# jonassibbesen/rpvg

Hardware: AMD Instinct MI355X
Metric: read-pairs quantified/sec (higher is better)
Workload: dtype f64

## Files before the change

rpvg_amd/csrc/bounded_search.hip:

```cpp

#include "common.hpp"
#include "search_plan.hpp"

#include <algorithm>
#include <cstdlib>
#include <map>
#include <memory>
#include <mutex>
#include <numeric>

using namespace rpvg_hip_detail;
using namespace rpvg_search;

namespace {
std::mutex g_search_gate_mutex;
const rpvg_hip_ctx * g_search_gate_owner = nullptr;
}

static bool searchLaunchesEarly() {
    static const bool early = RPVG_EXPERIMENT_ENV("RPVG_HIP_SEARCH_LAUNCH_EARLY") != nullptr;
    return early;
}

constexpr uint64_t kSearchGateRows = 1ull << 17;

static void searchGateEnter(rpvg_hip_ctx * ctx, hipStream_t stream, const uint64_t matrix_rows) {
    static const bool open_gate = RPVG_EXPERIMENT_ENV("RPVG_HIP_NO_SEARCH_GATE") != nullptr;
    ctx->search_gate_held = !open_gate && matrix_rows >= kSearchGateRows;
    if (!ctx->search_gate_held) return;
    hipEvent_t previous = nullptr;
    {
        std::lock_guard<std::mutex> lock(g_search_gate_mutex);
        if (g_search_gate_owner && g_search_gate_owner != ctx && g_search_gate_owner->device == ctx->device) {
            previous = g_search_gate_owner->search_done;
            (void) hipStreamWaitEvent(stream, previous, 0);
        }
    }
    if (previous && !searchLaunchesEarly()) (void) waitEvent(previous);
}

static void searchGateLeave(rpvg_hip_ctx * ctx, hipStream_t stream) {
    if (!ctx->search_gate_held) return;
    ctx->search_gate_held = false;
    std::lock_guard<std::mutex> lock(g_search_gate_mutex);
    (void) hipEventRecord(ctx->search_done, stream);
    g_search_gate_owner = ctx;
}

void searchGateForget(const rpvg_hip_ctx * ctx) {
    std::lock_guard<std::mutex> lock(g_search_gate_mutex);
    if (g_search_gate_owner == ctx) g_search_gate_owner = nullptr;
}

struct rpvg_hip_pair_posteriors {
    std::vector<uint64_t> pair_off;
    void * block = nullptr;
    bool block_pinned = false;
    const uint32_t * first = nullptr, * second = nullptr;
    const double * posterior = nullptr;
    ~rpvg_hip_pair_posteriors() {
        if (block && block_pinned) pinnedFree(block);
        else std::free(block);
    }
};

namespace {

constexpr uint32_t kLdsRows = 2048;
constexpr uint32_t kSmallRowLdsCols = 128;
constexpr uint32_t kRowLdsCols = 512;

// ... 1276 lines not shown
```

rpvg_amd/csrc/subset_em.hip:

```cpp

#include "common.hpp"
#include "subset_pack.hpp"

#include <cmath>
#include <memory>

using namespace rpvg_hip_detail;

namespace {

constexpr uint32_t kMaxSelected = 1024;

struct MergedList {
    const uint32_t * a;
    const uint32_t * b;
    uint32_t na, nb, i, j;
    __device__ __forceinline__ MergedList(const uint32_t * a_in, uint32_t na_in, const uint32_t * b_in, uint32_t nb_in)
        : a(a_in), b(b_in), na(na_in), nb(nb_in), i(0), j(0) {}
    __device__ __forceinline__ bool done() const { return i >= na && j >= nb; }
    __device__ __forceinline__ uint32_t next() {
        if (j >= nb || (i < na && a[i] <= b[j])) return a[i++];
        return b[j++];
    }
};

struct Columns {
    const uint64_t * group_path_off;
    const uint32_t * group_path;
    uint64_t first_column;
    __device__ __forceinline__ MergedList list(const uint32_t first, const uint32_t second) const {
        const uint64_t a0 = group_path_off[first_column + first], a1 = group_path_off[first_column + first + 1];
        const uint64_t b0 = group_path_off[first_column + second], b1 = group_path_off[first_column + second + 1];
        return MergedList(group_path + a0, static_cast<uint32_t>(a1 - a0), group_path + b0, static_cast<uint32_t>(b1 - b0));
    }
};
// ... 2 lines not shown
    while (!x.done() && !y.done()) {
        const uint32_t px = x.next(), py = y.next();
        if (px != py) return px < py ? -1 : 1;
    }
    if (x.done() && y.done()) return 0;
    return x.done() ? -1 : 1;
}

struct SelectArgs {
    uint32_t num_matrices;
    const uint32_t * pair_count;
    const uint64_t * pair_cap_off;
    const uint32_t * pair_first;
    const uint32_t * pair_second;
    const double * pair_value;
    const uint64_t * group_off;
    const uint64_t * group_path_off;
    const uint32_t * group_path;
    const uint32_t * cluster;
    const uint64_t * mat_rows;
    const uint64_t * cluster_row_off;
    const uint64_t * row_ent_off;
    const uint64_t * slot_off;
    double min_hap_prob;
    uint32_t segment_rows;
    uint32_t * slot_first;
    uint32_t * slot_second;
    double * slot_weight;
    uint32_t * slot_length;
    uint32_t * slot_columns;
    MatrixTotals * totals;
    SubsetHeader * header;
    uint32_t * big_matrices;
};

constexpr uint32_t kSmallSelected = 64;
constexpr uint32_t kSmallCachedPaths = 1024, kWideCachedPaths = 6144;

struct CachedColumns {
    const uint64_t * group_path_off;
    const uint32_t * paths;
    uint64_t first_column, base;
    __device__ __forceinline__ MergedList list(const uint32_t first, const uint32_t second) const {
        const uint64_t a0 = group_path_off[first_column + first], a1 = group_path_off[first_column + first + 1];
        const uint64_t b0 = group_path_off[first_column + second], b1 = group_path_off[first_column + second + 1];
        return MergedList(paths + (a0 - base), static_cast<uint32_t>(a1 - a0), paths + (b0 - base), static_cast<uint32_t>(b1 - b0));
    }
};

template <uint32_t CAP, uint32_t CACHE, int BLOCK>
__device__ __forceinline__ void selectSubsetsOfMatrix(const SelectArgs & args, const uint32_t m) {
    __shared__ uint32_t sel[CAP];
    __shared__ unsigned long long hash[CAP];
    __shared__ uint32_t length[CAP];
    __shared__ uint32_t leader[CAP];
    __shared__ double weight[CAP];
    __shared__ uint32_t order[CAP];
    __shared__ uint32_t cached_paths[CACHE];
    __shared__ uint32_t scratch[BLOCK / 64];
    __shared__ double sum_posterior;
    __shared__ unsigned long long red[3];
    __shared__ uint32_t n_retained;
    const uint32_t n_pairs = args.pair_count[m];
    const uint64_t base = args.pair_cap_off[m];
    const uint32_t * first = args.pair_first + base;
    const uint32_t * second = args.pair_second + base;
    const double * value = args.pair_value + base;
    const uint32_t k = args.cluster[m];
    MatrixTotals * out_totals = args.totals + m;
    const uint64_t col0 = args.group_off[m], col1 = args.group_off[m + 1];
    const uint64_t path0 = args.group_path_off[col0], path1 = args.group_path_off[col1];
    const bool cached = path1 - path0 <= CACHE;
    if (cached) {
        for (uint32_t i = threadIdx.x; i < path1 - path0; i += BLOCK) cached_paths[i] = args.group_path[path0 + i];
    }
    const CachedColumns columns{args.group_path_off, cached ? cached_paths : args.group_path, col0, cached ? path0 : 0};

    uint32_t n_sel = 0;
    for (uint32_t c = 0; c < n_pairs; c += BLOCK) {
        const uint32_t i = c + threadIdx.x;
        const uint32_t take = (i < n_pairs && value[i] >= args.min_hap_prob) ? 1u : 0u;
        uint32_t total;
        const uint32_t at = n_sel + blockExclusiveScan<BLOCK>(take, total, scratch);
        if (take && at < CAP) sel[at] = i;
        n_sel += total;
    }
    if (n_sel > CAP) {
        if (threadIdx.x == 0) {
            atomicAdd(&args.header->select_overflow, 1ull);
            *out_totals = MatrixTotals{0, 0, 0, 0, 0, 0};
        }
        return;
    }
    __syncthreads();
    if (threadIdx.x == 0) {
        double sum = 0;
        for (uint32_t s = 0; s < n_sel; ++s) sum += value[sel[s]];
        sum_posterior = sum;
        red[0] = red[1] = red[2] = 0;
        n_retained = 0;
    }
    for (uint32_t s = threadIdx.x; s < n_sel; s += BLOCK) {
        MergedList list = columns.list(first[sel[s]], second[sel[s]]);
        unsigned long long h = 1469598103934665603ull;
        uint32_t n = 0;
        while (!list.done()) {
            h = (h ^ list.next()) * 1099511628211ull;
            ++n;
        }
        hash[s] = h;
        length[s] = n;
    }
    __syncthreads();
    for (uint32_t s = threadIdx.x; s < n_sel; s += BLOCK) {
        uint32_t lead = s;
        for (uint32_t t = 0; t < s; ++t) {
            if (hash[t] == hash[s] && length[t] == length[s] &&
                compareLists(columns.list(first[sel[t]], second[sel[t]]), columns.list(first[sel[s]], second[sel[s]])) == 0) {
                lead = t;
                break;
            }
        }
        leader[s] = lead;
    }
    __syncthreads();
    for (uint32_t s = threadIdx.x; s < n_sel; s += BLOCK) {
        double w = 0;
        if (leader[s] == s) {
            for (uint32_t t = s; t < n_sel; ++t) {
                if (leader[t] == s) w += value[sel[t]];
            }
            w /= sum_posterior;
            if (w >= args.min_hap_prob) order[atomicAdd(&n_retained, 1u)] = s;
        }
        weight[s] = w;
    }
    __syncthreads();
    const uint32_t n_ret = n_retained;
    uint32_t padded = 1;
    while (padded < n_ret) padded <<= 1;
    for (uint32_t i = n_ret + threadIdx.x; i < padded; i += BLOCK) order[i] = 0xffffffffu;
    __syncthreads();
    auto before = [&](const uint32_t x, const uint32_t y) {
        if (x == 0xffffffffu) return false;
        if (y == 0xffffffffu) return true;
        return compareLists(columns.list(first[sel[x]], second[sel[x]]), columns.list(first[sel[y]], second[sel[y]])) < 0;
    };
    for (uint32_t size = 2; size <= padded; size <<= 1) {
        for (uint32_t stride = size >> 1; stride > 0; stride >>= 1) {
            for (uint32_t i = threadIdx.x; i < padded; i += BLOCK) {
                const uint32_t partner = i ^ stride;
                if (partner > i) {
                    const bool ascending = (i & size) == 0;
                    const uint32_t x = order[i], y = order[partner];
                    if (before(y, x) == ascending) {
                        order[i] = y;
                        order[partner] = x;
                    }
                }
            }
            __syncthreads();
        }
    }
    const uint64_t slot0 = args.slot_off[m];
    unsigned long long my_subsets = 0, my_length = 0, my_columns = 0;
    for (uint32_t rank = threadIdx.x; rank < n_ret; rank += BLOCK) {
        const uint32_t s = order[rank];
        uint32_t distinct = 0, previous = 0xffffffffu;
        MergedList walk = columns.list(first[sel[s]], second[sel[s]]);
        while (!walk.done()) {
            const uint32_t path = walk.next();
            distinct += (path != previous) ? 1u : 0u;
            previous = path;
        }
        args.slot_first[slot0 + rank] = first[sel[s]];
        args.slot_second[slot0 + rank] = second[sel[s]];
        args.slot_weight[slot0 + rank] = weight[s];
        args.slot_length[slot0 + rank] = length[s];
        args.slot_columns[slot0 + rank] = distinct;
        my_subsets += 1;
        my_length += length[s];
        my_columns += distinct;
    }
    if (my_subsets) {
        atomicAdd(&red[0], my_subsets);
        atomicAdd(&red[1], my_length);
        atomicAdd(&red[2], my_columns);
    }
    __syncthreads();
    if (threadIdx.x == 0) {
        const uint64_t r0 = args.cluster_row_off[k], r1 = args.cluster_row_off[k + 1];
        const unsigned long long rows = r1 - r0, entries = args.row_ent_off[r1] - args.row_ent_off[r0];
        *out_totals = MatrixTotals{red[0], red[1], red[2], red[0] * rows, red[0] * entries, red[0] * ((rows + args.segment_rows - 1) / args.segment_rows)};
    }
}

__global__ __launch_bounds__(64) void subsetSelectSmallKernel(const SelectArgs args) {
    const uint32_t m = blockIdx.x;
    if (m >= args.num_matrices) return;
    if (args.pair_count[m] > kSmallSelected) {
        if (threadIdx.x == 0) args.big_matrices[atomicAdd(&args.header->big_count, 1u)] = m;
        return;
    }
    selectSubsetsOfMatrix<kSmallSelected, kSmallCachedPaths, 64>(args, m);
}

__global__ __launch_bounds__(256) void subsetSelectWideKernel(const SelectArgs args) {
    const uint32_t count = args.header->big_count;
    for (uint32_t item = blockIdx.x; item < count; item += gridDim.x) {
        selectSubsetsOfMatrix<kMaxSelected, kWideCachedPaths, 256>(args, args.big_matrices[item]);
        __syncthreads();
    }
}

struct ExpandArgs {
    uint32_t num_matrices;
    const SubsetHeader * header;
    const MatrixTotals * totals;
    const MatrixTotals * bases;
    const uint64_t * slot_off;
    const uint32_t * slot_first;
    const uint32_t * slot_second;
    const double * slot_weight;
    const uint32_t * slot_length;
    const uint32_t * slot_columns;
    const uint64_t * group_off;
    const uint64_t * group_path_off;
    const uint32_t * group_path;
    const uint32_t * cluster;
    const uint64_t * cluster_row_off;
    const uint64_t * row_ent_off;
    uint32_t * sub_cluster;
    double * sub_weight;
    uint64_t * path_off;
    uint32_t * path;
    uint64_t * col_off;
    uint32_t * col_path;
    uint64_t * row_base;
    uint64_t * ent_base;
    uint64_t * seg_first;
    uint32_t * item_problem;
    uint32_t segment_rows;
    uint64_t * subset_off;
// ... 217 lines not shown
    if (tid == 0) set_count[m] = Q;
}

}


static int nestedSubsetEmAttempt(rpvg_hip_ctx * ctx, const rpvg_hip_batch * batch, const rpvg_hip_groups * groups,
                                 const uint32_t * column_counts, double min_rel_likelihood, double min_hap_prob,
                                 uint32_t max_em_its, double max_rel_em_conv, double collapse_precision,
                                 rpvg_hip_subset_em ** result_out, bool * did_not_fit, PairSearchWork & search, const bool second_attempt) {
    *did_not_fit = false;
    RPVG_REQUIRE(min_rel_likelihood > 0, "rpvg_hip_nested_subset_em: min_rel_likelihood must be positive");
    RPVG_REQUIRE(max_em_its > 0, "rpvg_hip_nested_subset_em: max_em_its must be positive");
    RPVG_REQUIRE(groups->batch == batch, "rpvg_hip_nested_subset_em: the matrices were built on another batch");
    const uint32_t M = groups->num_matrices;
    RPVG_REQUIRE(M == 0 || column_counts || groups->d_column_counts, "rpvg_hip_nested_subset_em: column_counts is NULL");
    std::unique_ptr<rpvg_hip_subset_em> res(new (std::nothrow) rpvg_hip_subset_em());
    if (!res) {
        setError("rpvg_hip_nested_subset_em: out of host memory");
        return RPVG_HIP_ERR_ALLOC;
    }
    res->num_matrices = M;

    const bool disabled = std::getenv("RPVG_HIP_NO_DEVICE_SUBSETS") != nullptr;
    if (disabled || !(min_hap_prob * kMaxSelected >= 1.0)) {
        setError("rpvg_hip_nested_subset_em: not taken (min_hap_prob %g admits more than %u subsets per cluster, or RPVG_HIP_NO_DEVICE_SUBSETS)",
                 min_hap_prob, kMaxSelected);
        return RPVG_HIP_ERR_UNSUPPORTED;
    }
    std::unique_ptr<HostScope> scope(new HostScope("subset em: bounds"));
    uint64_t slots = 0, lane_rows = 0, lane_entries = 0, lane_paths = 0, max_cluster_work = 0;
    uint32_t max_paths = 0;
    std::vector<uint64_t> slot_off(M + 1, 0);
    for (uint32_t m = 0; m < M; ++m) {
        const uint64_t G = groups->h_num_cols[m];
        slot_off[m + 1] = slot_off[m] + std::min<uint64_t>(G * (G + 1) / 2, kMaxSelected);
        const uint32_t k = groups->h_cluster[m];
        lane_rows += batch->h_cluster_row_off[k + 1] - batch->h_cluster_row_off[k];
        lane_entries += batch->h_cluster_ent_off[k + 1] - batch->h_cluster_ent_off[k];
        lane_paths += groups->h_num_paths[m];
        max_paths = std::max(max_paths, groups->h_num_paths[m]);
        max_cluster_work = std::max<uint64_t>(max_cluster_work, (batch->h_cluster_row_off[k + 1] - batch->h_cluster_row_off[k]) +
                                                                    (batch->h_cluster_ent_off[k + 1] - batch->h_cluster_ent_off[k]));
    }
    slots = slot_off[M];
    if (M > 0 && 8ull * (5ull * (static_cast<uint64_t>(max_paths) + 1) + 6) > 156 * 1024) {
        setError("rpvg_hip_nested_subset_em: not taken (a cluster with %u paths: EM vectors in global memory)", max_paths);
        return RPVG_HIP_ERR_UNSUPPORTED;
    }

    std::lock_guard<std::mutex> lock(ctx->mutex);
    RPVG_HIP_CHECK(hipSetDevice(ctx->device));
    hipStream_t st = ctx->stream;
    if (M == 0) {
        *result_out = res.release();
        return RPVG_HIP_OK;
    }
    SubsetEmHints & hints = ctx->subset_hints;
    auto planned = [](const double per_unit, const unsigned long long units, const double headroom) {
        return static_cast<unsigned long long>(std::ceil(per_unit * headroom * static_cast<double>(units)));
    };
    unsigned long long cap_subsets = std::min<unsigned long long>(slots, hints.subsets_per_matrix > 0 ? planned(hints.subsets_per_matrix, M, 1.25) + 256 : std::max<unsigned long long>(8ull * M, 16384));
    unsigned long long cap_length = std::max<unsigned long long>(planned(hints.list_per_path, lane_paths, 2.0), std::max<unsigned long long>(8 * lane_paths, 1u << 20));
    unsigned long long cap_rows = hints.rows_per_row > 0 ? planned(hints.rows_per_row, lane_rows, 1.25) + 65536 : 8 * lane_rows;
    unsigned long long cap_entries = hints.entries_per_entry > 0 ? planned(hints.entries_per_entry, lane_entries, 1.25) + 65536 : 8 * lane_entries;
    if (hints.retry) {
        cap_subsets = std::min<unsigned long long>(slots, std::max(cap_subsets, hints.retry_subsets + 64));
        cap_length = std::max(cap_length, hints.retry_list_length + 64);
        cap_rows = std::max(cap_rows, hints.retry_rows + 64);
        cap_entries = std::max(cap_entries, hints.retry_entries + 64);
        hints.retry = false;
    }
    const unsigned long long cap_columns = cap_length;
    const unsigned long long cap_items = cap_rows / emFillSegmentRows() + cap_subsets;

    scope.reset(new HostScope("subset em: search + kernels queued"));
    const size_t header_room = 256;
    int rc = RPVG_HIP_OK;
    if (!second_attempt) {
        search.extra_u64 = slot_off.data();
        search.extra_u64_count = M + 1;
        search.extra_zero_bytes = header_room + emQueuesBytes();
        rc = queuePairSearch(ctx, groups, column_counts, min_rel_likelihood, search);
        if (rc != RPVG_HIP_OK) return rc;
    } else {
        const hipError_t zeroed = zeroAsync(search.d_extra_zero.ptr, search.extra_zero_bytes, st);
        if (zeroed != hipSuccess) {
            setError("rpvg_hip_nested_subset_em: %s", hipGetErrorString(zeroed));
            return RPVG_HIP_ERR_RUNTIME;
        }
    }

    hipError_t e = hipSuccess;
    auto ok = [&](hipError_t r) { if (e == hipSuccess) e = r; return e == hipSuccess; };
    const uint64_t * d_slot_off = search.d_extra_u64.ptr;
    SubsetHeader * header = reinterpret_cast<SubsetHeader *>(search.d_extra_zero.ptr);
    static_assert(sizeof(SubsetHeader) <= 256, "room for the header");
    DeviceBuffer<uint32_t> d_slot_first, d_slot_second, d_slot_length, d_slot_columns;
    DeviceBuffer<double> d_slot_weight;
    DeviceBuffer<unsigned char> d_totals, d_bases, d_packed;
    ok(d_slot_first.alloc(slots));
    ok(d_slot_second.alloc(slots));
    ok(d_slot_length.alloc(slots));
    ok(d_slot_columns.alloc(slots));
    ok(d_slot_weight.alloc(slots));
    ok(d_totals.alloc(sizeof(MatrixTotals) * M));
    ok(d_bases.alloc(sizeof(MatrixTotals) * M));
    DeviceBuffer<uint32_t> d_big_matrices;
    ok(d_big_matrices.alloc(M));
    DeviceBuffer<uint32_t> d_sub_cluster, d_path, d_col_path, d_iters, d_kept_rows, d_kept_entries;
    DeviceBuffer<double> d_sub_weight, d_abund, d_noise, d_total;
    DeviceBuffer<uint64_t> d_path_off, d_col_off, d_row_base, d_ent_base, d_subset_off, d_seg_first;
    DeviceBuffer<uint32_t> d_item_problem;
    ok(d_sub_cluster.alloc(cap_subsets));
    ok(d_sub_weight.alloc(cap_subsets));
    ok(d_path_off.alloc(cap_subsets + 1));
    ok(d_col_off.alloc(cap_subsets + 1));
    ok(d_row_base.alloc(cap_subsets));
    ok(d_ent_base.alloc(cap_subsets));
    ok(d_subset_off.alloc(M + 1));
    ok(d_seg_first.alloc(cap_subsets + 1));
    ok(d_item_problem.alloc(cap_items));
    ok(d_path.alloc(cap_length));
    ok(d_col_path.alloc(cap_columns));
    ok(d_abund.alloc(cap_columns));
    ok(d_noise.alloc(cap_subsets));
    ok(d_total.alloc(cap_subsets));
    ok(d_iters.alloc(cap_subsets));
    ok(d_kept_rows.alloc(cap_subsets));
    ok(d_kept_entries.alloc(cap_subsets));
    const size_t packed_capacity = packedLayout(M, cap_subsets, cap_length, cap_columns).bytes;
    ok(d_packed.alloc(packed_capacity));
    const bool merge_here = batch->path_group_id.ptr != nullptr && max_paths < (1u << kMergePathBits) - 2;
    DeviceBuffer<unsigned long long> d_merge_key;
    DeviceBuffer<uint32_t> d_merge_pos;
    DeviceBuffer<double> d_merge_a0, d_merge_a1;
    if (merge_here) {
        ok(d_merge_key.alloc(2 * cap_length + 2));
        ok(d_merge_pos.alloc(2 * cap_length + 2));
        ok(d_merge_a0.alloc(cap_length));
        ok(d_merge_a1.alloc(cap_length));
    }
// ... 9 lines not shown
        if (header_here) (void) hipEventDestroy(header_here);
        return (e == hipErrorOutOfMemory) ? RPVG_HIP_ERR_ALLOC : RPVG_HIP_ERR_RUNTIME;
    }
    MatrixTotals * totals = reinterpret_cast<MatrixTotals *>(d_totals.ptr);
    MatrixTotals * bases = reinterpret_cast<MatrixTotals *>(d_bases.ptr);

    std::unique_ptr<HostScope> part_scope(new HostScope("subset em: select + offsets + expand queued"));
    int span = ctx->spanBegin(FAM_BUILD);
    SelectArgs sa;
    sa.num_matrices = M;
    sa.pair_count = search.d_tail.ptr;
    sa.pair_cap_off = search.d_pair_cap_off.ptr;
    sa.pair_first = search.d_out_first.ptr;
    sa.pair_second = search.d_out_second.ptr;
    sa.pair_value = search.d_out_value.ptr;
    sa.group_off = groups->d_group_off;
    sa.group_path_off = groups->d_group_path_off;
    sa.group_path = groups->d_group_path;
    sa.cluster = groups->d_cluster;
    sa.mat_rows = groups->mat_rows.ptr;
    sa.cluster_row_off = batch->cluster_row_off.ptr;
    sa.row_ent_off = batch->row_ent_off.ptr;
    sa.slot_off = d_slot_off;
    sa.min_hap_prob = min_hap_prob;
    sa.segment_rows = emFillSegmentRows();
    sa.slot_first = d_slot_first.ptr;
    sa.slot_second = d_slot_second.ptr;
    sa.slot_weight = d_slot_weight.ptr;
    sa.slot_length = d_slot_length.ptr;
    sa.slot_columns = d_slot_columns.ptr;
    sa.totals = totals;
    sa.header = header;
    sa.big_matrices = d_big_matrices.ptr;
    subsetSelectSmallKernel<<<dim3(M), dim3(64), 0, st>>>(sa);
    subsetSelectWideKernel<<<dim3(std::min<uint32_t>(M, 128)), dim3(256), 0, st>>>(sa);
    const bool check_build = !groups->build_checked && groups->build_error_flag.ptr;
    OffsetsArgs oa;
    oa.pair_count = search.d_tail.ptr;
    oa.log_evals = reinterpret_cast<const unsigned long long *>(search.d_tail.ptr + search.evals_word);
    oa.build_error = check_build ? groups->build_error_flag.ptr : nullptr;
    oa.num_matrices = M;
    oa.totals = totals;
    oa.bases = bases;
    oa.header = header;
    oa.cap_subsets = cap_subsets;
    oa.cap_length = cap_length;
    oa.cap_columns = cap_columns;
    oa.cap_rows = cap_rows;
    oa.cap_entries = cap_entries;
    oa.cap_items = cap_items;
    oa.seg_first = d_seg_first.ptr;
    oa.path_off = d_path_off.ptr;
    oa.col_off = d_col_off.ptr;
    subsetOffsetsKernel<<<dim3(1), dim3(1024), 0, st>>>(oa);
    SubsetHeader * h_header = static_cast<SubsetHeader *>(pinned_header);
    ok(hipMemcpyAsync(h_header, header, sizeof(SubsetHeader), hipMemcpyDeviceToHost, st));
    ok(hipEventRecord(header_here, st));
    ExpandArgs ea;
    ea.num_matrices = M;
    ea.header = header;
    ea.totals = totals;
    ea.bases = bases;
    ea.slot_off = d_slot_off;
    ea.slot_first = d_slot_first.ptr;
    ea.slot_second = d_slot_second.ptr;
    ea.slot_weight = d_slot_weight.ptr;
    ea.slot_length = d_slot_length.ptr;
    ea.slot_columns = d_slot_columns.ptr;
// ... 129 lines not shown
        return RPVG_HIP_ERR_INVALID;
    }
    groups->build_checked = true;
    if (got.overflow) {
        (void) hipStreamSynchronize(st);
        setError("rpvg_hip_nested_subset_em: not taken (%llu subsets, %llu rows, %llu entries, %llu selected-diplotype overflows: over the reserved "
                 "capacity)", got.subsets, got.rows, got.entries, got.select_overflow);
        if (!got.select_overflow) {
            hints.retry = true;
            hints.retry_subsets = got.subsets;
            hints.retry_list_length = std::max(got.list_length, got.columns);
            hints.retry_rows = got.rows;
            hints.retry_entries = got.entries;
            *did_not_fit = true;
        }
        return RPVG_HIP_ERR_UNSUPPORTED;
    }
    scope.reset(new HostScope("subset em: wait for the EM + download"));
    const uint64_t S = got.subsets;
    const PackedLayout lay = packedLayout(M, S, got.list_length, got.columns);
    if (pinnedAlloc(&res->block, std::max<size_t>(lay.bytes, 64)) != hipSuccess) {
        (void) hipStreamSynchronize(st);
        setError("rpvg_hip_nested_subset_em: out of page-locked host memory");
        return RPVG_HIP_ERR_ALLOC;
    }
    unsigned char * host = static_cast<unsigned char *>(res->block);
    ok(hipMemcpyAsync(host, d_packed.ptr, lay.bytes, hipMemcpyDeviceToHost, st));
    ok(waitStream(st));
    if (e != hipSuccess) {
        setError("rpvg_hip_nested_subset_em: %s", hipGetErrorString(e));
        return RPVG_HIP_ERR_RUNTIME;
    }
    accountPairSearch(ctx, groups, search, got.log_evals, got.kept_pairs);

    rpvg_hip_subset_em_view & v = res->view;
    v.num_matrices = M;
    v.subset_off = reinterpret_cast<const uint64_t *>(host + lay.subset_off);
    v.weight = reinterpret_cast<const double *>(host + lay.weight);
    v.path_off = reinterpret_cast<const uint64_t *>(host + lay.path_off);
    v.path = reinterpret_cast<const uint32_t *>(host + lay.path);
    v.col_off = reinterpret_cast<const uint64_t *>(host + lay.col_off);
    v.col_path = reinterpret_cast<const uint32_t *>(host + lay.col_path);
    v.abundances = reinterpret_cast<const double *>(host + lay.abundances);
    v.noise_count = reinterpret_cast<const double *>(host + lay.noise);
    v.total_count = reinterpret_cast<const double *>(host + lay.total);
    v.iterations = reinterpret_cast<const uint32_t *>(host + lay.iterations);
    if (merge_here) {
        if (*reinterpret_cast<const uint32_t *>(host + lay.merge_flags)) {
            setError("rpvg_hip_nested_subset_em: a diplotype's path subset holds more than two paths of one transcript (PathInfo::group_id): "
                     "the reference asserts against it (src/path_abundance_estimator.cpp:722)");
            return RPVG_HIP_ERR_INVALID;
        }
        v.set_count = reinterpret_cast<const uint32_t *>(host + lay.set_count);
        v.cluster_noise_count = reinterpret_cast<const double *>(host + lay.cluster_noise);
        v.set_first = reinterpret_cast<const uint32_t *>(host + lay.set_first);
        v.set_second = reinterpret_cast<const uint32_t *>(host + lay.set_second);
        v.set_posterior = reinterpret_cast<const double *>(host + lay.set_posterior);
        v.set_abundance = reinterpret_cast<const double *>(host + lay.set_abund);
    }
    res->num_subsets = S;
    accountEmSolve(ctx, static_cast<uint32_t>(S), v.col_off, reinterpret_cast<const uint32_t *>(host + lay.kept_rows),
                   reinterpret_cast<const uint32_t *>(host + lay.kept_entries), v.iterations);
    *result_out = res.release();
    return RPVG_HIP_OK;
}

// ... 28 lines not shown
```

rpvg_amd/hip.py:

```python
from __future__ import annotations

import ctypes as C
import os
from typing import List, Optional, Sequence, Tuple

import numpy as np

from .batch import CClusterBatch, ClusterBatch

_HERE = os.path.dirname(os.path.abspath(__file__))
LIB_PATH = os.path.join(_HERE, "csrc", "librpvg_hip.so")

EXPORTS = [
    "rpvg_hip_device_count", "rpvg_hip_create", "rpvg_hip_create_uploader", "rpvg_hip_destroy", "rpvg_hip_last_error", "rpvg_hip_synchronize",
    "rpvg_hip_device_info", "rpvg_hip_malloc", "rpvg_hip_free", "rpvg_hip_memcpy_h2d", "rpvg_hip_memcpy_d2h",
    "rpvg_hip_batch_upload", "rpvg_hip_batch_free", "rpvg_hip_em_solve", "rpvg_hip_em_dense",
    "rpvg_hip_dense_from_cluster", "rpvg_hip_groups_build", "rpvg_hip_groups_free", "rpvg_hip_groups_collapse_info", "rpvg_hip_group_loglik",
    "rpvg_hip_synth_dense_cluster", "rpvg_hip_stats_get", "rpvg_hip_stats_reset", "rpvg_hip_stats_intervals", "rpvg_hip_em_kernel_name",
    "rpvg_hip_gibbs_read_counts", "rpvg_hip_min_path_cover", "rpvg_hip_min_path_cover_any", "rpvg_hip_cover_limits", "rpvg_hip_bounded_pair_posteriors", "rpvg_hip_pair_posteriors_get", "rpvg_hip_pair_posteriors_free",
    "rpvg_hip_em_dense_sharded", "rpvg_hip_synth_dense_rows", "rpvg_hip_synth_dense_cluster_batch", "rpvg_hip_comm_unique_id", "rpvg_hip_comm_init",
    "rpvg_hip_comm_destroy", "rpvg_hip_comm_allreduce_sum_f64", "rpvg_hip_comm_init_all", "rpvg_hip_gather", "rpvg_hip_host_register", "rpvg_hip_host_unregister", "rpvg_hip_group_conditionals",
    "rpvg_hip_group_gibbs", "rpvg_hip_group_gibbs_polyploid", "rpvg_hip_gibbs_sets_get", "rpvg_hip_gibbs_sets_free",
    "rpvg_hip_alignments_upload", "rpvg_hip_alignments_free", "rpvg_hip_read_rows_build", "rpvg_hip_read_rows_to_batch",
    "rpvg_hip_read_rows_view", "rpvg_hip_read_rows_sizes", "rpvg_hip_read_rows_free", "rpvg_hip_path_clusters", "rpvg_hip_debug_log",
# ... 32 lines not shown

class CEmProblems(C.Structure):
    _fields_ = [("num_problems", C.c_uint32), ("cluster", C.c_void_p), ("col_off", C.c_void_p), ("col_path", C.c_void_p),
                ("collapse_precision", C.c_double)]


class CEmResults(C.Structure):
    _fields_ = [("abundances", C.c_void_p), ("noise_count", C.c_void_p), ("total_count", C.c_void_p),
                ("iterations", C.c_void_p)]


class CGroupSpec(C.Structure):
    _fields_ = [("num_matrices", C.c_uint32), ("cluster", C.c_void_p), ("group_off", C.c_void_p),
                ("group_path_off", C.c_void_p), ("group_path", C.c_void_p), ("normalise", C.c_int32),
                ("collapse_precision", C.c_double)]


class CGibbsSpec(C.Structure):
    _fields_ = [("num_problems", C.c_uint32), ("group_size", C.c_uint32), ("matrix", C.c_void_p), ("num_chains", C.c_void_p),
                ("num_burn_its", C.c_void_p), ("num_gibbs_its", C.c_void_p), ("log_freq", C.c_void_p), ("num_generators", C.c_uint32),
                ("generator_problem_off", C.c_void_p), ("generator_problem", C.c_void_p), ("generator_words", C.c_void_p)]


class CGibbsSetsView(C.Structure):
    _fields_ = [("num_problems", C.c_uint32), ("group_size", C.c_uint32), ("set_off", C.POINTER(C.c_uint64)),
                ("first", C.POINTER(C.c_uint32)), ("second", C.POINTER(C.c_uint32)), ("count", C.POINTER(C.c_uint32)),
                ("words_consumed", C.POINTER(C.c_uint64)), ("generator_state", C.POINTER(C.c_uint32)), ("rounds", C.c_uint32),
                ("conditionals", C.c_uint64), ("members", C.POINTER(C.c_uint32))]


class CPairPosteriorsView(C.Structure):
    _fields_ = [("num_matrices", C.c_uint32), ("pair_off", C.POINTER(C.c_uint64)), ("first", C.POINTER(C.c_uint32)),
                ("second", C.POINTER(C.c_uint32)), ("posterior", C.POINTER(C.c_double))]


class CSubsetEmSetsView(C.Structure):
    _fields_ = [("num_matrices", C.c_uint32), ("group_size", C.c_uint32), ("subset_off", C.POINTER(C.c_uint64)),
                ("weight", C.POINTER(C.c_double)), ("path_off", C.POINTER(C.c_uint64)), ("path", C.POINTER(C.c_uint32)),
                ("col_off", C.POINTER(C.c_uint64)), ("col_path", C.POINTER(C.c_uint32)), ("abundances", C.POINTER(C.c_double)),
                ("noise_count", C.POINTER(C.c_double)), ("total_count", C.POINTER(C.c_double)), ("iterations", C.POINTER(C.c_uint32)),
                ("retained_off", C.POINTER(C.c_uint64)), ("retained_rank", C.POINTER(C.c_uint64)),
                ("retained_posterior", C.POINTER(C.c_double)), ("set_count", C.POINTER(C.c_uint32)),
                ("cluster_noise_count", C.POINTER(C.c_double)), ("set_size", C.POINTER(C.c_uint32)), ("set_member", C.POINTER(C.c_uint32)),
                ("set_posterior", C.POINTER(C.c_double)), ("set_abundance", C.POINTER(C.c_double))]


class CIndependentSpec(C.Structure):
    _fields_ = [("num_clusters", C.c_uint32), ("matrix_off", C.c_void_p), ("group_size", C.c_uint32), ("column_counts", C.c_void_p),
                ("log_freq", C.c_void_p), ("min_hap_prob", C.c_double), ("max_em_its", C.c_uint32), ("max_rel_em_conv", C.c_double),
                ("collapse_precision", C.c_double), ("generator_words", C.c_void_p), ("keep_draws", C.c_int32)]


class CSubsetEmIndependentView(C.Structure):
    _fields_ = [("num_clusters", C.c_uint32), ("group_size", C.c_uint32), ("num_samples", C.c_uint32), ("subset_off", C.POINTER(C.c_uint64)),
                ("weight", C.POINTER(C.c_double)), ("path_off", C.POINTER(C.c_uint64)), ("path", C.POINTER(C.c_uint32)),
                ("col_off", C.POINTER(C.c_uint64)), ("col_path", C.POINTER(C.c_uint32)), ("abundances", C.POINTER(C.c_double)),
                ("noise_count", C.POINTER(C.c_double)), ("total_count", C.POINTER(C.c_double)), ("iterations", C.POINTER(C.c_uint32)),
                ("set_count", C.POINTER(C.c_uint32)), ("cluster_noise_count", C.POINTER(C.c_double)), ("set_size", C.POINTER(C.c_uint32)),
                ("set_member", C.POINTER(C.c_uint32)), ("set_posterior", C.POINTER(C.c_double)), ("set_abundance", C.POINTER(C.c_double)),
                ("sample_count", C.POINTER(C.c_uint32)), ("words_consumed", C.POINTER(C.c_uint64)), ("generator_state", C.POINTER(C.c_uint32))]


class CIndependentLimits(C.Structure):
    _fields_ = [("max_group_size", C.c_uint32), ("max_samples", C.c_uint32), ("max_transcript_sets", C.c_uint64), ("words_per_draw", C.c_uint32),
                ("state_words", C.c_uint32), ("max_work_bytes", C.c_uint64)]

# ... 431 lines not shown
        if mem.ndim == 1:
            mem = mem.reshape(len(mt), -1)
        width = mem.shape[1]
        out = np.zeros(len(mt), dtype=np.float64)
        flag = None if add_rowmax is None else np.ascontiguousarray(add_rowmax, dtype=np.uint8)
        _check(lib().rpvg_hip_group_loglik(self.ctx.handle, self.handle, C.c_uint32(len(mt)), C.c_void_p(mt.ctypes.data),
                                           C.c_void_p(mem.ctypes.data), C.c_uint32(width), C.c_double(divisor),
                                           C.c_void_p(flag.ctypes.data if flag is not None else None),
                                           C.c_void_p(out.ctypes.data)), "rpvg_hip_group_loglik")
        return out

    def conditionals(self, matrix, others, width: int, divisor: float, num_cols) -> List[np.ndarray]:
        mt = np.ascontiguousarray(matrix, dtype=np.uint32)
        oth = np.ascontiguousarray(others, dtype=np.uint32).reshape(len(mt), max(width - 1, 0))
        sizes = [int(num_cols[int(m)]) for m in mt]
        out = np.zeros(sum(sizes), dtype=np.float64)
        _check(lib().rpvg_hip_group_conditionals(self.ctx.handle, self.handle, C.c_uint32(len(mt)), C.c_void_p(mt.ctypes.data),
                                                 C.c_void_p(oth.ctypes.data if oth.size else None), C.c_uint32(width),
                                                 C.c_double(divisor), C.c_void_p(out.ctypes.data)),
               "rpvg_hip_group_conditionals")
        return np.split(out, np.cumsum(sizes)[:-1]) if sizes else []

    def full_posteriors(self, matrix, group_size: int, log_freq, num_cols) -> List[np.ndarray]:
        mt = np.ascontiguousarray(matrix, dtype=np.uint32)
        lf = np.ascontiguousarray(np.concatenate([np.asarray(x, dtype=np.float64) for x in log_freq]) if len(log_freq) else np.zeros(0))
        sizes = [int(lib().rpvg_hip_full_set_count(C.c_uint32(int(num_cols[int(m)])), C.c_uint32(group_size))) for m in mt]
        out = np.zeros(sum(s for s in sizes if s <= 0x7fffffff), dtype=np.float64)
        _check(lib().rpvg_hip_group_full_posteriors(self.ctx.handle, self.handle, C.c_uint32(len(mt)), C.c_void_p(mt.ctypes.data),
                                                    C.c_uint32(group_size), C.c_void_p(lf.ctypes.data if lf.size else None),
                                                    C.c_void_p(out.ctypes.data if out.size else None)),
               "rpvg_hip_group_full_posteriors")
        return np.split(out, np.cumsum(sizes)[:-1]) if sizes else []

    def nested_full_subset_em(self, group_size: int, log_freq, min_hap_prob: float, max_em_its: int = 10000, max_rel_em_conv: float = 1e-3,
                              collapse_precision: float = 0.0) -> dict:
        lf = np.ascontiguousarray(np.concatenate([np.asarray(x, dtype=np.float64) for x in log_freq]) if len(log_freq) else np.zeros(0))
        h = C.c_void_p()
        _check(lib().rpvg_hip_nested_full_subset_em(self.ctx.handle, self.batch.handle, self.handle, C.c_uint32(group_size),
                                                    C.c_void_p(lf.ctypes.data if lf.size else None), C.c_double(float(min_hap_prob)),
                                                    C.c_uint32(max_em_its), C.c_double(float(max_rel_em_conv)),
                                                    C.c_double(float(collapse_precision)), C.byref(h)), "rpvg_hip_nested_full_subset_em")
        try:
            v = CSubsetEmSetsView()
            _check(lib().rpvg_hip_subset_em_get_sets(h, C.byref(v)), "rpvg_hip_subset_em_get_sets")
            M, g = int(v.num_matrices), int(v.group_size)

            def take(pointer, n, dtype, shape=None):
                if n == 0 or not pointer:
                    return np.zeros(shape if shape is not None else (0,), dtype=dtype)
                a = np.ctypeslib.as_array(pointer, shape=(n,)).copy()
                return a.reshape(shape) if shape is not None else a

            out = {"num_matrices": M, "group_size": g}
            if M == 0:
                out.update({"subset_off": np.zeros(1, np.uint64), "path_off": np.zeros(1, np.uint64), "col_off": np.zeros(1, np.uint64),
                            "retained_off": np.zeros(1, np.uint64)})
                for name, dtype in (("weight", np.float64), ("path", np.uint32), ("col_path", np.uint32), ("abundances", np.float64),
                                    ("noise_count", np.float64), ("total_count", np.float64), ("iterations", np.uint32),
                                    ("retained_rank", np.uint64), ("retained_posterior", np.float64), ("set_count", np.uint32),
                                    ("cluster_noise_count", np.float64), ("set_size", np.uint32), ("set_posterior", np.float64)):
                    out[name] = np.zeros(0, dtype)
                out["set_member"] = np.zeros((0, g), np.uint32)
                out["set_abundance"] = np.zeros((0, g), np.float64)
                return out
            out["subset_off"] = take(v.subset_off, M + 1, np.uint64)
            S = int(out["subset_off"][-1])
# ... 445 lines not shown
```

Measured before the change: 2.534 billion.

## Rewrite wide subset selection with hash-table dedup and staged merged lists

Adds a dedicated wide-matrix selection routine that stages list offsets in shared memory, replaces the quadratic leader search with a shared hash table keyed on hash and length, accumulates weights over a compacted follower list, and sorts using cached list heads plus pre-merged path lists. This targets the O(n^2) leader and weight loops and the repeated global merges during the bitonic sort. The old path stays available through an environment switch or when offsets would overflow. It also adds optional timing stamps and a Python binding, and it raises shared-memory use in the wide kernel, which may lower occupancy.

New measurement: 2.556 billion, median of 2. No clear change (+0.8%).

```diff
diff --git a/rpvg_amd/csrc/bounded_search.hip b/rpvg_amd/csrc/bounded_search.hip
--- a/rpvg_amd/csrc/bounded_search.hip
+++ b/rpvg_amd/csrc/bounded_search.hip
@@ -36,7 +36,10 @@
             (void) hipStreamWaitEvent(stream, previous, 0);
         }
     }
-    if (previous && !searchLaunchesEarly()) (void) waitEvent(previous);
+    if (previous && !searchLaunchesEarly()) {
+        HostScope wait_scope("search: wait for the search in front");
+        (void) waitEvent(previous);
+    }
 }
 
 static void searchGateLeave(rpvg_hip_ctx * ctx, hipStream_t stream) {
diff --git a/rpvg_amd/csrc/subset_em.hip b/rpvg_amd/csrc/subset_em.hip
--- a/rpvg_amd/csrc/subset_em.hip
+++ b/rpvg_amd/csrc/subset_em.hip
@@ -1,6 +1,7 @@
 
 #include "common.hpp"
 #include "subset_pack.hpp"
+#include "subset_select_plan.hpp"
 
 #include <cmath>
 #include <memory>
@@ -69,7 +70,19 @@
     MatrixTotals * totals;
     SubsetHeader * header;
     uint32_t * big_matrices;
+    unsigned long long * stamps;
 };
+
+constexpr uint32_t kStampItems = 16, kStampWords = 32, kStampTimes = 16;
+enum : uint32_t { STAMP_MATRIX = 0, STAMP_PAIRS, STAMP_SELECTED, STAMP_RETAINED, STAMP_ENTRIES, STAMP_FOLLOWERS };
+enum : uint32_t { AT_START = 0, AT_SELECTED, AT_STAGED, AT_HASHED, AT_LEADERS, AT_WEIGHTS, AT_SORTED, AT_SLOTS };
+#ifdef RPVG_HIP_EXPERIMENTS
+#define SELECT_NOTE(word, value) do { if (stamp && threadIdx.x == 0) stamp[word] = (value); } while (0)
+#define SELECT_STAMP(phase) SELECT_NOTE(kStampTimes + (phase), wall_clock64())
+#else
+#define SELECT_NOTE(word, value) do { } while (0)
+#define SELECT_STAMP(phase) do { } while (0)
+#endif
 
 constexpr uint32_t kSmallSelected = 64;
 constexpr uint32_t kSmallCachedPaths = 1024, kWideCachedPaths = 6144;
@@ -86,7 +99,7 @@
 };
 
 template <uint32_t CAP, uint32_t CACHE, int BLOCK>
-__device__ __forceinline__ void selectSubsetsOfMatrix(const SelectArgs & args, const uint32_t m) {
+__device__ __forceinline__ void selectSubsetsOfMatrix(const SelectArgs & args, const uint32_t m, unsigned long long * stamp = nullptr) {
     __shared__ uint32_t sel[CAP];
     __shared__ unsigned long long hash[CAP];
     __shared__ uint32_t length[CAP];
@@ -108,6 +121,10 @@
     const uint64_t col0 = args.group_off[m], col1 = args.group_off[m + 1];
     const uint64_t path0 = args.group_path_off[col0], path1 = args.group_path_off[col1];
     const bool cached = path1 - path0 <= CACHE;
+    SELECT_NOTE(STAMP_MATRIX, m + 1);
+    SELECT_NOTE(STAMP_PAIRS, n_pairs);
+    SELECT_NOTE(STAMP_ENTRIES, path1 - path0);
+    SELECT_STAMP(AT_START);
     if (cached) {
         for (uint32_t i = threadIdx.x; i < path1 - path0; i += BLOCK) cached_paths[i] = args.group_path[path0 + i];
     }
@@ -122,6 +139,7 @@
         if (take && at < CAP) sel[at] = i;
         n_sel += total;
     }
+    SELECT_NOTE(STAMP_SELECTED, n_sel);
     if (n_sel > CAP) {
         if (threadIdx.x == 0) {
             atomicAdd(&args.header->select_overflow, 1ull);
@@ -130,6 +148,7 @@
         return;
     }
     __syncthreads();
+    SELECT_STAMP(AT_SELECTED);
     if (threadIdx.x == 0) {
         double sum = 0;
         for (uint32_t s = 0; s < n_sel; ++s) sum += value[sel[s]];
@@ -137,6 +156,7 @@
         red[0] = red[1] = red[2] = 0;
         n_retained = 0;
     }
+    SELECT_STAMP(AT_STAGED);
     for (uint32_t s = threadIdx.x; s < n_sel; s += BLOCK) {
         MergedList list = columns.list(first[sel[s]], second[sel[s]]);
         unsigned long long h = 1469598103934665603ull;
@@ -149,6 +169,7 @@
         length[s] = n;
     }
     __syncthreads();
+    SELECT_STAMP(AT_HASHED);
     for (uint32_t s = threadIdx.x; s < n_sel; s += BLOCK) {
         uint32_t lead = s;
         for (uint32_t t = 0; t < s; ++t) {
@@ -161,6 +182,7 @@
         leader[s] = lead;
     }
     __syncthreads();
+    SELECT_STAMP(AT_LEADERS);
     for (uint32_t s = threadIdx.x; s < n_sel; s += BLOCK) {
         double w = 0;
         if (leader[s] == s) {
@@ -173,7 +195,9 @@
         weight[s] = w;
     }
     __syncthreads();
+    SELECT_STAMP(AT_WEIGHTS);
     const uint32_t n_ret = n_retained;
+    SELECT_NOTE(STAMP_RETAINED, n_ret);
     uint32_t padded = 1;
     while (padded < n_ret) padded <<= 1;
     for (uint32_t i = n_ret + threadIdx.x; i < padded; i += BLOCK) order[i] = 0xffffffffu;
@@ -199,6 +223,7 @@
             __syncthreads();
         }
     }
+    SELECT_STAMP(AT_SORTED);
     const uint64_t slot0 = args.slot_off[m];
     unsigned long long my_subsets = 0, my_length = 0, my_columns = 0;
     for (uint32_t rank = threadIdx.x; rank < n_ret; rank += BLOCK) {
@@ -230,6 +255,7 @@
         const unsigned long long rows = r1 - r0, entries = args.row_ent_off[r1] - args.row_ent_off[r0];
         *out_totals = MatrixTotals{red[0], red[1], red[2], red[0] * rows, red[0] * entries, red[0] * ((rows + args.segment_rows - 1) / args.segment_rows)};
     }
+    SELECT_STAMP(AT_SLOTS);
 }
 
 __global__ __launch_bounds__(64) void subsetSelectSmallKernel(const SelectArgs args) {
@@ -242,10 +268,277 @@
     selectSubsetsOfMatrix<kSmallSelected, kSmallCachedPaths, 64>(args, m);
 }
 
+__global__ __launch_bounds__(256) void subsetSelectWideSerialKernel(const SelectArgs args) {
+    const uint32_t count = args.header->big_count;
+    for (uint32_t item = blockIdx.x; item < count; item += gridDim.x) {
+        selectSubsetsOfMatrix<kMaxSelected, kWideCachedPaths, 256>(args, args.big_matrices[item],
+                                                                   args.stamps && item < kStampItems ? args.stamps + item * kStampWords : nullptr);
+        __syncthreads();
+    }
+}
+
+constexpr uint32_t kWideTable = 2 * kMaxSelected, kNoPair = 0xffffffffu;
+constexpr uint32_t kWideMergedPaths = 8192;
+
+struct StagedLists {
+    const uint32_t * paths;
+    const uint32_t * a_at;
+    const uint32_t * a_len;
+    const uint32_t * b_at;
+    const uint32_t * b_len;
+    __device__ __forceinline__ MergedList list(const uint32_t s) const {
+        return MergedList(paths + a_at[s], a_len[s], paths + b_at[s], b_len[s]);
+    }
+};
+
+template <int BLOCK>
+__device__ __forceinline__ void selectSubsetsOfWideMatrix(const SelectArgs & args, const uint32_t m, unsigned long long * stamp) {
+    constexpr uint32_t CAP = kMaxSelected, CACHE = kWideCachedPaths;
+    __shared__ uint32_t sel[CAP];
+    __shared__ double posterior[CAP];
+    __shared__ uint32_t a_at[CAP], a_len[CAP], b_at[CAP], b_len[CAP];
+    __shared__ unsigned long long hash[CAP];
+    __shared__ unsigned long long head[CAP];
+    __shared__ uint32_t length[CAP];
+    __shared__ uint32_t distinct[CAP];
+    __shared__ uint32_t leader[CAP];
+    __shared__ uint32_t follower[CAP];
+    __shared__ double weight[CAP];
+    __shared__ uint32_t order[CAP];
+    __shared__ uint32_t table[kWideTable];
+    __shared__ uint32_t merged_at[CAP];
+    __shared__ uint32_t merged[kWideMergedPaths + 4];
+    __shared__ uint32_t cached_paths[CACHE];
+    __shared__ uint32_t scratch[BLOCK / 64];
+    __shared__ double sum_posterior;
+    __shared__ unsigned long long red[3];
+    __shared__ uint32_t n_retained;
+    const uint32_t n_pairs = args.pair_count[m];
+    const uint64_t base = args.pair_cap_off[m];
+    const uint32_t * first = args.pair_first + base;
+    const uint32_t * second = args.pair_second + base;
+    const double * value = args.pair_value + base;
+    const uint32_t k = args.cluster[m];
+    MatrixTotals * out_totals = args.totals + m;
+    const uint64_t col0 = args.group_off[m], col1 = args.group_off[m + 1];
+    const uint64_t path0 = args.group_path_off[col0], path1 = args.group_path_off[col1];
+    const bool cached = path1 - path0 <= CACHE;
+    SELECT_NOTE(STAMP_MATRIX, m + 1);
+    SELECT_NOTE(STAMP_PAIRS, n_pairs);
+    SELECT_NOTE(STAMP_ENTRIES, path1 - path0);
+    SELECT_STAMP(AT_START);
+    if (cached) {
+        for (uint32_t i = threadIdx.x; i < path1 - path0; i += BLOCK) cached_paths[i] = args.group_path[path0 + i];
+    }
+    for (uint32_t i = threadIdx.x; i < kWideTable; i += BLOCK) table[i] = kNoPair;
+    const StagedLists lists{cached ? cached_paths : args.group_path + path0, a_at, a_len, b_at, b_len};
+
+    uint32_t n_sel = 0;
+    for (uint32_t c = 0; c < n_pairs; c += BLOCK) {
+        const uint32_t i = c + threadIdx.x;
+        const uint32_t take = (i < n_pairs && value[i] >= args.min_hap_prob) ? 1u : 0u;
+        uint32_t total;
+        const uint32_t at = n_sel + blockExclusiveScan<BLOCK>(take, total, scratch);
+        if (take && at < CAP) sel[at] = i;
+        n_sel += total;
+    }
+    SELECT_NOTE(STAMP_SELECTED, n_sel);
+    if (n_sel > CAP) {
+        if (threadIdx.x == 0) {
+            atomicAdd(&args.header->select_overflow, 1ull);
+            *out_totals = MatrixTotals{0, 0, 0, 0, 0, 0};
+        }
+        return;
+    }
+    __syncthreads();
+    SELECT_STAMP(AT_SELECTED);
+    for (uint32_t s = threadIdx.x; s < n_sel; s += BLOCK) {
+        const uint32_t i = sel[s];
+        const uint64_t ca = col0 + first[i], cb = col0 + second[i];
+        const uint64_t a0 = args.group_path_off[ca], a1 = args.group_path_off[ca + 1];
+        const uint64_t b0 = args.group_path_off[cb], b1 = args.group_path_off[cb + 1];
+        posterior[s] = value[i];
+        a_at[s] = static_cast<uint32_t>(a0 - path0);
+        a_len[s] = static_cast<uint32_t>(a1 - a0);
+        b_at[s] = static_cast<uint32_t>(b0 - path0);
+        b_len[s] = static_cast<uint32_t>(b1 - b0);
+    }
+    __syncthreads();
+    SELECT_STAMP(AT_STAGED);
+    if (threadIdx.x == BLOCK - 1) {
+        double sum = 0;
+        for (uint32_t s = 0; s < n_sel; ++s) sum += posterior[s];
+        sum_posterior = sum;
+        red[0] = red[1] = red[2] = 0;
+        n_retained = 0;
+    }
+    for (uint32_t s = threadIdx.x; s < n_sel; s += BLOCK) {
+        MergedList list = lists.list(s);
+        unsigned long long h = 1469598103934665603ull, front = 0;
+        uint32_t n = 0, different = 0, previous = 0xffffffffu;
+        while (!list.done()) {
+            const uint32_t path = list.next();
+            h = (h ^ path) * 1099511628211ull;
+            if (n < 2) front = (front << 32) | path;
+            different += (path != previous) ? 1u : 0u;
+            previous = path;
+            ++n;
+        }
+        hash[s] = h;
+        head[s] = front;
+        length[s] = n;
+        distinct[s] = different;
+    }
+    __syncthreads();
+    SELECT_STAMP(AT_HASHED);
+    auto same_key = [&](const uint32_t s, const uint32_t t) { return hash[t] == hash[s] && length[t] == length[s]; };
+    auto first_entry = [&](const uint32_t s) { return static_cast<uint32_t>(hash[s] ^ (hash[s] >> 32)) & (kWideTable - 1); };
+    for (uint32_t s = threadIdx.x; s < n_sel; s += BLOCK) {
+        for (uint32_t entry = first_entry(s);; entry = (entry + 1) & (kWideTable - 1)) {
+            const uint32_t seen = atomicCAS(&table[entry], kNoPair, s);
+            if (seen == kNoPair) break;
+            if (same_key(s, seen)) {
+                atomicMin(&table[entry], s);
+                break;
+            }
+        }
+    }
+    __syncthreads();
+    for (uint32_t s = threadIdx.x; s < n_sel; s += BLOCK) {
+        uint32_t entry = first_entry(s);
+        while (!same_key(s, table[entry])) entry = (entry + 1) & (kWideTable - 1);
+        const uint32_t lowest = table[entry];
+        uint32_t lead = s;
+        if (lowest != s) {
+            if (compareLists(lists.list(lowest), lists.list(s)) == 0) {
+                lead = lowest;
+            } else {
+                for (uint32_t t = lowest + 1; t < s; ++t) {
+                    if (same_key(s, t) && compareLists(lists.list(t), lists.list(s)) == 0) {
+                        lead = t;
+                        break;
+                    }
+                }
+            }
+        }
+        leader[s] = lead;
+    }
+    __syncthreads();
+    SELECT_STAMP(AT_LEADERS);
+    uint32_t n_follow = 0;
+    for (uint32_t c = 0; c < n_sel; c += BLOCK) {
+        const uint32_t s = c + threadIdx.x;
+        const uint32_t led = (s < n_sel && leader[s] != s) ? 1u : 0u;
+        uint32_t total;
+        const uint32_t at = n_follow + blockExclusiveScan<BLOCK>(led, total, scratch);
+        if (led) follower[at] = s;
+        n_follow += total;
+    }
+    SELECT_NOTE(STAMP_FOLLOWERS, n_follow);
+    __syncthreads();
+    for (uint32_t s = threadIdx.x; s < n_sel; s += BLOCK) {
+        double w = 0;
+        if (leader[s] == s) {
+            w += posterior[s];
+            for (uint32_t f = 0; f < n_follow; ++f) {
+                const uint32_t t = follower[f];
+                if (leader[t] == s) w += posterior[t];
+            }
+            w /= sum_posterior;
+            if (w >= args.min_hap_prob) order[atomicAdd(&n_retained, 1u)] = s;
+        }
+        weight[s] = w;
+    }
+    __syncthreads();
+    SELECT_STAMP(AT_WEIGHTS);
+    const uint32_t n_ret = n_retained;
+    SELECT_NOTE(STAMP_RETAINED, n_ret);
+    uint32_t padded = 1;
+    while (padded < n_ret) padded <<= 1;
+    for (uint32_t i = n_ret + threadIdx.x; i < padded; i += BLOCK) order[i] = kNoPair;
+    uint32_t merged_total = 0;
+    for (uint32_t c = 0; c < n_ret; c += BLOCK) {
+        const uint32_t rank = c + threadIdx.x;
+        const uint32_t s = rank < n_ret ? order[rank] : kNoPair;
+        uint32_t total;
+        const uint32_t at = merged_total + blockExclusiveScan<BLOCK>(s != kNoPair ? length[s] : 0u, total, scratch);
+        if (s != kNoPair) merged_at[s] = at;
+        merged_total += total;
+    }
+    const bool written_out = merged_total <= kWideMergedPaths;
+    __syncthreads();
+    if (written_out) {
+        for (uint32_t rank = threadIdx.x; rank < n_ret; rank += BLOCK) {
+            const uint32_t s = order[rank];
+            uint32_t * out = merged + merged_at[s];
+            MergedList list = lists.list(s);
+            while (!list.done()) *out++ = list.next();
+        }
+    }
+    __syncthreads();
+    auto before = [&](const uint32_t x, const uint32_t y) {
+        if (x == kNoPair) return false;
+        if (y == kNoPair) return true;
+        if (length[x] >= 2 && length[y] >= 2 && head[x] != head[y]) return head[x] < head[y];
+        if (!written_out) return compareLists(lists.list(x), lists.list(y)) < 0;
+        const uint32_t nx = length[x], ny = length[y], n = nx < ny ? nx : ny;
+        const uint32_t * px = merged + merged_at[x], * py = merged + merged_at[y];
+        for (uint32_t i = 0; i < n; i += 4) {
+            const uint32_t x0 = px[i], x1 = px[i + 1], x2 = px[i + 2], x3 = px[i + 3];
+            const uint32_t y0 = py[i], y1 = py[i + 1], y2 = py[i + 2], y3 = py[i + 3];
+            if (x0 != y0) return x0 < y0;
+            if (i + 1 < n && x1 != y1) return x1 < y1;
+            if (i + 2 < n && x2 != y2) return x2 < y2;
+            if (i + 3 < n && x3 != y3) return x3 < y3;
+        }
+        return nx < ny;
+    };
+    for (uint32_t size = 2; size <= padded; size <<= 1) {
+        for (uint32_t stride = size >> 1; stride > 0; stride >>= 1) {
+            for (uint32_t pair = threadIdx.x; pair < padded / 2; pair += BLOCK) {
+                const uint32_t i = ((pair & ~(stride - 1)) << 1) | (pair & (stride - 1)), partner = i | stride;
+                const bool ascending = (i & size) == 0;
+                const uint32_t x = order[i], y = order[partner];
+                if (before(y, x) == ascending) {
+                    order[i] = y;
+                    order[partner] = x;
+                }
+            }
+            __syncthreads();
+        }
+    }
+    SELECT_STAMP(AT_SORTED);
+    const uint64_t slot0 = args.slot_off[m];
+    unsigned long long my_subsets = 0, my_length = 0, my_columns = 0;
+    for (uint32_t rank = threadIdx.x; rank < n_ret; rank += BLOCK) {
+        const uint32_t s = order[rank];
+        args.slot_first[slot0 + rank] = first[sel[s]];
+        args.slot_second[slot0 + rank] = second[sel[s]];
+        args.slot_weight[slot0 + rank] = weight[s];
+        args.slot_length[slot0 + rank] = length[s];
+        args.slot_columns[slot0 + rank] = distinct[s];
+        my_subsets += 1;
+        my_length += length[s];
+        my_columns += distinct[s];
+    }
+    if (my_subsets) {
+        atomicAdd(&red[0], my_subsets);
+        atomicAdd(&red[1], my_length);
+        atomicAdd(&red[2], my_columns);
+    }
+    __syncthreads();
+    if (threadIdx.x == 0) {
+        const uint64_t r0 = args.cluster_row_off[k], r1 = args.cluster_row_off[k + 1];
+        const unsigned long long rows = r1 - r0, entries = args.row_ent_off[r1] - args.row_ent_off[r0];
+        *out_totals = MatrixTotals{red[0], red[1], red[2], red[0] * rows, red[0] * entries, red[0] * ((rows + args.segment_rows - 1) / args.segment_rows)};
+    }
+    SELECT_STAMP(AT_SLOTS);
+}
+
 __global__ __launch_bounds__(256) void subsetSelectWideKernel(const SelectArgs args) {
     const uint32_t count = args.header->big_count;
     for (uint32_t item = blockIdx.x; item < count; item += gridDim.x) {
-        selectSubsetsOfMatrix<kMaxSelected, kWideCachedPaths, 256>(args, args.big_matrices[item]);
+        selectSubsetsOfWideMatrix<256>(args, args.big_matrices[item], args.stamps && item < kStampItems ? args.stamps + item * kStampWords : nullptr);
         __syncthreads();
     }
 }
@@ -529,8 +822,11 @@
     uint64_t slots = 0, lane_rows = 0, lane_entries = 0, lane_paths = 0, max_cluster_work = 0;
     uint32_t max_paths = 0;
     std::vector<uint64_t> slot_off(M + 1, 0);
+    SelectWidePlan select_plan;
+    select_plan.asked(std::getenv("RPVG_HIP_SELECT_SERIAL") != nullptr);
     for (uint32_t m = 0; m < M; ++m) {
         const uint64_t G = groups->h_num_cols[m];
+        select_plan.matrix(groups->h_num_cols[m], groups->h_num_paths[m]);
         slot_off[m + 1] = slot_off[m] + std::min<uint64_t>(G * (G + 1) / 2, kMaxSelected);
         const uint32_t k = groups->h_cluster[m];
         lane_rows += batch->h_cluster_row_off[k + 1] - batch->h_cluster_row_off[k];
@@ -541,6 +837,7 @@
                                                                     (batch->h_cluster_ent_off[k + 1] - batch->h_cluster_ent_off[k]));
     }
     slots = slot_off[M];
+    const bool serial_select = select_plan.serial;
     if (M > 0 && 8ull * (5ull * (static_cast<uint64_t>(max_paths) + 1) + 6) > 156 * 1024) {
         setError("rpvg_hip_nested_subset_em: not taken (a cluster with %u paths: EM vectors in global memory)", max_paths);
         return RPVG_HIP_ERR_UNSUPPORTED;
@@ -605,6 +902,11 @@
     ok(d_bases.alloc(sizeof(MatrixTotals) * M));
     DeviceBuffer<uint32_t> d_big_matrices;
     ok(d_big_matrices.alloc(M));
+    DeviceBuffer<unsigned long long> d_stamps;
+    if (RPVG_EXPERIMENT_ENV("RPVG_HIP_SELECT_STAMPS")) {
+        ok(d_stamps.alloc(kStampItems * kStampWords));
+        if (e == hipSuccess) ok(zeroAsync(d_stamps.ptr, sizeof(unsigned long long) * kStampItems * kStampWords, st));
+    }
     DeviceBuffer<uint32_t> d_sub_cluster, d_path, d_col_path, d_iters, d_kept_rows, d_kept_entries;
     DeviceBuffer<double> d_sub_weight, d_abund, d_noise, d_total;
     DeviceBuffer<uint64_t> d_path_off, d_col_off, d_row_base, d_ent_base, d_subset_off, d_seg_first;
@@ -680,8 +982,13 @@
     sa.totals = totals;
     sa.header = header;
     sa.big_matrices = d_big_matrices.ptr;
+    sa.stamps = d_stamps.ptr;
     subsetSelectSmallKernel<<<dim3(M), dim3(64), 0, st>>>(sa);
-    subsetSelectWideKernel<<<dim3(std::min<uint32_t>(M, 128)), dim3(256), 0, st>>>(sa);
+    if (serial_select) {
+        subsetSelectWideSerialKernel<<<dim3(std::min<uint32_t>(M, 128)), dim3(256), 0, st>>>(sa);
+    } else {
+        subsetSelectWideKernel<<<dim3(std::min<uint32_t>(M, 128)), dim3(256), 0, st>>>(sa);
+    }
     const bool check_build = !groups->build_checked && groups->build_error_flag.ptr;
     OffsetsArgs oa;
     oa.pair_count = search.d_tail.ptr;
@@ -877,6 +1184,22 @@
         return RPVG_HIP_ERR_RUNTIME;
     }
     accountPairSearch(ctx, groups, search, got.log_evals, got.kept_pairs);
+    if (d_stamps.ptr) {
+        std::vector<unsigned long long> stamps(kStampItems * kStampWords);
+        if (hipMemcpy(stamps.data(), d_stamps.ptr, sizeof(unsigned long long) * stamps.size(), hipMemcpyDeviceToHost) == hipSuccess) {
+            std::fprintf(stderr, "[select stamps] %s role, %u wide matrices of %u\n", serial_select ? "serial" : "wide", got.big_count, M);
+            for (uint32_t item = 0; item < kStampItems; ++item) {
+                const unsigned long long * w = stamps.data() + item * kStampWords, * t = w + kStampTimes;
+                if (!w[STAMP_MATRIX]) continue;
+                auto us = [&](const uint32_t from, const uint32_t to) { return t[to] >= t[from] ? 0.01 * static_cast<double>(t[to] - t[from]) : -1.0; };
+                std::fprintf(stderr, "[select stamps] matrix %llu pairs %llu selected %llu retained %llu led-by-another %llu path-entries %llu | us: select %.1f "
+                             "stage-or-sum %.1f hash %.1f leaders %.1f weights %.1f sort %.1f slots %.1f total %.1f\n", w[STAMP_MATRIX] - 1, w[STAMP_PAIRS],
+                             w[STAMP_SELECTED], w[STAMP_RETAINED], w[STAMP_FOLLOWERS], w[STAMP_ENTRIES], us(AT_START, AT_SELECTED), us(AT_SELECTED, AT_STAGED),
+                             us(AT_STAGED, AT_HASHED), us(AT_HASHED, AT_LEADERS), us(AT_LEADERS, AT_WEIGHTS), us(AT_WEIGHTS, AT_SORTED), us(AT_SORTED, AT_SLOTS),
+                             us(AT_START, AT_SLOTS));
+            }
+        }
+    }
 
     rpvg_hip_subset_em_view & v = res->view;
     v.num_matrices = M;
diff --git a/rpvg_amd/csrc/subset_select_plan.hpp b/rpvg_amd/csrc/subset_select_plan.hpp
--- /dev/null
+++ b/rpvg_amd/csrc/subset_select_plan.hpp
@@ -0,0 +1,17 @@
+#pragma once
+
+#include <cstdint>
+
+namespace rpvg_hip_detail {
+
+inline bool selectWideOffsetsFit(const uint32_t columns, const uint32_t paths) {
+    return static_cast<uint64_t>(columns) * static_cast<uint64_t>(paths) <= 0xffffffffull;
+}
+
+struct SelectWidePlan {
+    bool serial = false;
+    void asked(const bool serial_wanted) { serial = serial || serial_wanted; }
+    void matrix(const uint32_t columns, const uint32_t paths) { serial = serial || !selectWideOffsetsFit(columns, paths); }
+};
+
+}
diff --git a/rpvg_amd/hip.py b/rpvg_amd/hip.py
--- a/rpvg_amd/hip.py
+++ b/rpvg_amd/hip.py
@@ -88,6 +88,15 @@
 class CPairPosteriorsView(C.Structure):
     _fields_ = [("num_matrices", C.c_uint32), ("pair_off", C.POINTER(C.c_uint64)), ("first", C.POINTER(C.c_uint32)),
                 ("second", C.POINTER(C.c_uint32)), ("posterior", C.POINTER(C.c_double))]
+
+
+class CSubsetEmView(C.Structure):
+    _fields_ = [("num_matrices", C.c_uint32), ("subset_off", C.POINTER(C.c_uint64)), ("weight", C.POINTER(C.c_double)),
+                ("path_off", C.POINTER(C.c_uint64)), ("path", C.POINTER(C.c_uint32)), ("col_off", C.POINTER(C.c_uint64)),
+                ("col_path", C.POINTER(C.c_uint32)), ("abundances", C.POINTER(C.c_double)), ("noise_count", C.POINTER(C.c_double)),
+                ("total_count", C.POINTER(C.c_double)), ("iterations", C.POINTER(C.c_uint32)), ("set_count", C.POINTER(C.c_uint32)),
+                ("cluster_noise_count", C.POINTER(C.c_double)), ("set_first", C.POINTER(C.c_uint32)), ("set_second", C.POINTER(C.c_uint32)),
+                ("set_posterior", C.POINTER(C.c_double)), ("set_abundance", C.POINTER(C.c_double))]
 
 
 class CSubsetEmSetsView(C.Structure):
@@ -585,6 +594,38 @@
                "rpvg_hip_group_full_posteriors")
         return np.split(out, np.cumsum(sizes)[:-1]) if sizes else []
 
+    def nested_subset_em(self, column_counts, min_rel_likelihood: float, min_hap_prob: float, max_em_its: int = 10000,
+                         max_rel_em_conv: float = 1e-3, collapse_precision: float = 0.0) -> dict:
+        cc = np.ascontiguousarray(column_counts, dtype=np.uint32)
+        h = C.c_void_p()
+        _check(lib().rpvg_hip_nested_subset_em(self.ctx.handle, self.batch.handle, self.handle, C.c_void_p(cc.ctypes.data),
+                                               C.c_double(float(min_rel_likelihood)), C.c_double(float(min_hap_prob)), C.c_uint32(max_em_its),
+                                               C.c_double(float(max_rel_em_conv)), C.c_double(float(collapse_precision)), C.byref(h)),
+               "rpvg_hip_nested_subset_em")
+        try:
+            v = CSubsetEmView()
+            _check(lib().rpvg_hip_subset_em_get(h, C.byref(v)), "rpvg_hip_subset_em_get")
+            M = int(v.num_matrices)
+
+            def take(pointer, n, dtype):
+                return np.ctypeslib.as_array(pointer, shape=(n,)).copy() if n and pointer else np.zeros(0, dtype=dtype)
+
+            out = {"num_matrices": M, "subset_off": take(v.subset_off, M + 1, np.uint64) if M else np.zeros(1, np.uint64)}
+            S = int(out["subset_off"][-1])
+            out["path_off"] = take(v.path_off, S + 1, np.uint64) if M else np.zeros(1, np.uint64)
+            out["col_off"] = take(v.col_off, S + 1, np.uint64) if M else np.zeros(1, np.uint64)
+            L, Cn = int(out["path_off"][-1]), int(out["col_off"][-1])
+            out["weight"] = take(v.weight, S, np.float64)
+            out["path"] = take(v.path, L, np.uint32)
+            out["col_path"] = take(v.col_path, Cn, np.uint32)
+            out["abundances"] = take(v.abundances, Cn, np.float64)
+            out["noise_count"] = take(v.noise_count, S, np.float64)
+            out["total_count"] = take(v.total_count, S, np.float64)
+            out["iterations"] = take(v.iterations, S, np.uint32)
+            return out
+        finally:
+            lib().rpvg_hip_subset_em_free(h)
+
     def nested_full_subset_em(self, group_size: int, log_freq, min_hap_prob: float, max_em_its: int = 10000, max_rel_em_conv: float = 1e-3,
                               collapse_precision: float = 0.0) -> dict:
         lf = np.ascontiguousarray(np.concatenate([np.asarray(x, dtype=np.float64) for x in log_freq]) if len(log_freq) else np.zeros(0))
```
